# AI4quantum/qiskit-gym

Hardware: AMD Instinct MI355X
Metric: env-steps/sec (whole node), CliffordGym 16q x 65536 envs/GPU; bit-exact vs CPU (higher is better)
Workload: dtype u32

## Files before the change

### qiskit_gym_amd/csrc/kernels_qm.hip

```cpp
#include <cstdlib>

#include "device_common.hpp"
#include "qgym_plan.hpp"
#include "qm_step1.hpp"

namespace qg {


template <int NXP, bool HAS_Z>
struct QmRows {
    static constexpr int R = HAS_Z ? 2 * NXP : NXP;
    static constexpr int G = R / 4;
    static constexpr int xs(int j) { return HAS_Z ? 2 * j : j; }
    static constexpr int zs(int j) { return 2 * j + 1; }
    uint32_t r[R];
};

template <int NXP, bool HAS_Z>
__device__ inline void qm_load(const uint4 *tile, uint32_t lane, QmRows<NXP, HAS_Z> &s) {
#pragma unroll
    for (int g = 0; g < QmRows<NXP, HAS_Z>::G; ++g) {
        const uint4 q = tile[g * 64 + lane];
        s.r[4 * g + 0] = q.x; s.r[4 * g + 1] = q.y; s.r[4 * g + 2] = q.z; s.r[4 * g + 3] = q.w;
    }
// ... 202 lines not shown
        v[i] = i < R ? 1u << i : 0u;
    }
    uint32_t singular = 0;
#pragma unroll 1
    for (int col = 0; col < R; ++col) {
        uint32_t pm = 0, pv = 0;
#pragma unroll
        for (int k = 0; k < 32; ++k) {
            pm = (k == col) ? m[k] : pm;
            pv = (k == col) ? v[k] : pv;
        }
        uint32_t need = ((pm >> col) & 1u) - 1u;
#pragma unroll
        for (int r = 0; r < 32; ++r) {
            const uint32_t t = (r > col && r < R) ? (need & (0u - ((m[r] >> col) & 1u))) : 0u;
            pm ^= m[r] & t;
            pv ^= v[r] & t;
            need &= ~t;
        }
        singular |= need;
#pragma unroll
        for (int r = 0; r < 32; ++r) {
            const uint32_t t = (r != col && r < R) ? (0u - ((m[r] >> col) & 1u)) : 0u;
            m[r] = (r == col) ? pm : (m[r] ^ (pm & t));
            v[r] = (r == col) ? pv : (v[r] ^ (pv & t));
        }
    }
    if (singular) return false;
#pragma unroll
    for (int i = 0; i < 32; ++i) {
        const bool pad = i < R && (uint32_t)(i % NXP) >= N;
        if (pad) v[i] = 0;
    }
    if constexpr (HAS_Z) {
        qm_from_slot_space<NXP>(s, N, v);
    } else {
#pragma unroll
        for (int i = 0; i < R; ++i) s.r[i] = v[i];
    }
    return true;
}

template <int NXP>
__device__ inline void qm_symplectic_inverse(QmRows<NXP, true> &s, uint32_t N) {
    uint32_t m[32], c[32];
    qm_to_slot_space<NXP>(s, N, m);
    qm_symplectic_candidate<NXP>(m, c);
    qm_from_slot_space<NXP>(s, N, c);
}

template <int NXP>
__device__ inline bool qm_check_symplectic(const QmRows<NXP, true> &s, uint32_t N) {
    uint32_t m[32], c[32];
    qm_to_slot_space<NXP>(s, N, m);
    qm_symplectic_candidate<NXP>(m, c);
    return qm_is_inverse<NXP>(m, c, N);
}

template <int NXP, bool HAS_Z, bool FEAT, bool SEQ, bool INV = false, bool GJ = false>
__global__ __launch_bounds__(256) void qm_step_kernel(StepArgs a) {
    using Rows = QmRows<NXP, HAS_Z>;
    const uint64_t env = (uint64_t)blockIdx.x * blockDim.x + threadIdx.x;
    const uint32_t lane = threadIdx.x & (QG_WAVE - 1);
    const bool valid = env < a.B;
    const bool act64 = a.flags & F_ACT64;
    uint4 *tile = reinterpret_cast<uint4 *>(a.state) + (env >> 6) * (uint64_t)(Rows::G * 64);

    if (!valid) return;
    int64_t act = load_action(a.actions, env, act64);
    Rows s;
    qm_load<NXP, HAS_Z>(tile, lane, s);
    int32_t depth = a.depth[env];
    uint32_t iflags = INV ? a.inverted[env] : 0u;

    uint32_t dirty = 0;
    bool solved = false;
    float reward = 0.0f;
    uint32_t fault = 0;
    int32_t sol_n = (FEAT && (a.flags & F_TRACK)) ? a.sol_len[env * 2] : 0;
    int32_t sol_b = (FEAT && INV && (a.flags & F_TRACK)) ? a.sol_len[env * 2 + 1] : 0;

    const uint32_t T = SEQ ? a.T : 1u;
    for (uint32_t t = 0; t < T; ++t) {
        if (SEQ && t) act = load_action(a.actions, (uint64_t)t * a.B + env, act64);
        const bool in_range = act >= 0 && act < (int64_t)a.num_actions;
        GateEntry g = {QM_IDENTITY << 10, 0.0f};
        if (in_range) g = a.gates[act];
        float penalty = g.penalty;
        if (FEAT && (a.flags & F_LAYERS) && in_range)
            penalty = layers_penalty(layer_rec(a.layers, env, 2 * a.N + 2), a.N, a.descs[act], a.w);

        dirty |= qm_apply<NXP, HAS_Z>(s, g.ops);

        if (FEAT && (a.flags & F_TRACK)) {
            if ((uint32_t)(sol_n + sol_b) < a.sol_cap) {
                const bool inv_frame = INV && (iflags & QM_FLAG_INVERTED);
                sol_at(a, env, (uint32_t)(sol_n + sol_b)) = sol_word_framed(act, inv_frame);
                if (inv_frame) ++sol_b;
                else ++sol_n;
            } else {
                fault |= 8u;
            }
        }
        depth = depth > 0 ? depth - 1 : 0;
        if constexpr (INV) {
            const uint32_t coin = a.coins ? a.coins[(uint64_t)t * a.B + env]
                                          : (uint32_t)(rng_draw(a.seed ^ 0x636F696Eull, a.env_base + env, step_clock(a) + t) >> 63);
            if (coin & 1u) {
                bool fast = false;
                if constexpr (HAS_Z) {
                    if (iflags & QM_FLAG_SYMPLECTIC) {
                        qm_symplectic_inverse<NXP>(s, a.N);
                        fast = true;
                    }
                }
                if (fast) {
                    iflags ^= QM_FLAG_INVERTED;
                    dirty = 0xFFFFFFFFu;
                } else if constexpr (GJ) {
                    if (qm_gauss_jordan<NXP, HAS_Z>(s, a.N)) {
                        iflags ^= QM_FLAG_INVERTED;
                        dirty = 0xFFFFFFFFu;
                    } else {
                        fault |= QG_FAULT_SINGULAR;
                    }
                } else {
                    fault |= QG_FAULT_BAD_STATE;
                }
            }
        }
        solved = qm_solved<NXP, HAS_Z>(s, a.N);
        const float achieved = solved ? 1.0f : 0.0f;
        reward = achieved - penalty;
        if (SEQ && a.rewards_seq) a.rewards_seq[(uint64_t)t * a.B + env] = reward;
        if (SEQ && a.dones_seq) a.dones_seq[(uint64_t)t * a.B + env] = (uint8_t)(depth == 0 || solved);
    }

#pragma unroll
    for (int g = 0; g < Rows::G; ++g)
        if ((dirty >> g) & 1u) tile[g * 64 + lane] = make_uint4(s.r[4 * g], s.r[4 * g + 1], s.r[4 * g + 2], s.r[4 * g + 3]);
    a.depth[env] = depth;
    a.reward[env] = reward;
    a.done[env] = (uint8_t)(depth == 0 || solved);
    a.success[env] = (uint8_t)solved;
    if (FEAT && (a.flags & F_TRACK)) {
        a.sol_len[env * 2] = sol_n;
        if (INV) a.sol_len[env * 2 + 1] = sol_b;
    }
    if (INV) a.inverted[env] = (uint8_t)iflags;
    if ((FEAT || INV) && fault) atomicOr(&a.error[env], fault);
    if (a.bad) a.bad[env] = qm_badmask<NXP, HAS_Z>(s, a.N);
}

template <int NXP, bool FEAT, bool LIST = false, bool DENSE = false>
__global__ __launch_bounds__(256) void qm_inv2_kernel(StepArgs a) {
    KernelClock kclk(a.kclk, a.kclk_waves);
    const uint64_t tid = (uint64_t)blockIdx.x * blockDim.x + threadIdx.x;
    __shared__ uint32_t dense_rows[DENSE ? 4 : 1][DENSE ? 32 * 33 : 1];
    uint32_t *dl = DENSE ? dense_rows[threadIdx.x >> 6] : nullptr;
    QG_PREFETCH_STEP_ARGS(a);
    bool whole = false;
    if constexpr (LIST || DENSE) {
        bool fin = false;
        if ((tid >> 1) < a.B) fin = qm_inv2_body<NXP / 2, FEAT, DENSE>(a, NXP / 2, tid >> 1, (uint32_t)tid & 1u, nullptr, dl, &whole);
        if constexpr (DENSE) qm_inv2_dense_flush(a.dense, dl, (tid - (threadIdx.x & 63u)) >> 1, whole);
        if constexpr (LIST) done_mask_store_pairs(a.done_mask, a.B, fin, tid, a.done_epoch);
    } else {
        if ((tid >> 1) >= a.B) return;
        (void)qm_inv2_body<NXP / 2, FEAT, DENSE>(a, NXP / 2, tid >> 1, (uint32_t)tid & 1u, nullptr, dl, &whole);
    }
}


template <int NXP, bool HAS_Z, bool ACT64>
__global__ __launch_bounds__(256) void qm_fused_lds_kernel(StepArgs a) {
    using Rows = QmRows<NXP, HAS_Z>;
    __shared__ uint32_t lds_rows[4][Rows::R][QG_WAVE];
    const uint64_t env = (uint64_t)blockIdx.x * blockDim.x + threadIdx.x;
    const uint32_t lane = threadIdx.x & (QG_WAVE - 1);
    if (env >= a.B) return;
    uint32_t (*rows)[QG_WAVE] = lds_rows[threadIdx.x >> 6];
    uint4 *tile = reinterpret_cast<uint4 *>(a.state) + (env >> 6) * (uint64_t)(Rows::G * 64);
    uint32_t bad;
    {
        Rows s;
        qm_load<NXP, HAS_Z>(tile, lane, s);
        bad = qm_badmask<NXP, HAS_Z>(s, a.N);
#pragma unroll
        for (int k = 0; k < Rows::R; ++k) rows[k][lane] = s.r[k];
    }
    int32_t depth = a.depth[env];
    const uint32_t zb = 1u << a.N;
    float reward = 0.0f;
    bool solved = bad == 0;
    auto load_act = [&](uint32_t t) -> int64_t {
        const uint64_t i = (uint64_t)(t < a.T ? t : a.T - 1u) * a.B + env;
        const int64_t v = ACT64 ? reinterpret_cast<const int64_t *>(a.actions)[i] : (int64_t) reinterpret_cast<const int32_t *>(a.actions)[i];
        return t < a.T ? v : -1;
    };
    auto load_gate = [&](int64_t act, GateEntry &g) {
        const bool ok = act >= 0 && act < (int64_t)a.num_actions;
        const GateEntry e = a.gates[ok ? act : 0];
        g.ops = ok ? e.ops : (QM_IDENTITY << 10);
        g.penalty = ok ? e.penalty : 0.0f;
    };
    auto step = [&](uint32_t t, const GateEntry &g) {
        if (t >= a.T) return;
        const uint32_t q0 = g.ops & 31u, q1 = (g.ops >> 5) & 31u, m = (g.ops >> 10) & 0xFFFFu;
        if (m != QM_IDENTITY) {
            const uint32_t sx0 = HAS_Z ? 2u * q0 : q0, sx1 = HAS_Z ? 2u * q1 : q1;
            const uint32_t x0 = rows[sx0][lane], x1 = rows[sx1][lane];
            const uint32_t z0 = HAS_Z ? rows[sx0 + 1u][lane] : 0u, z1 = HAS_Z ? rows[sx1 + 1u][lane] : 0u;
            auto mix = [&](uint32_t k) -> uint32_t {
                const uint32_t b = m >> (4 * k);
                uint32_t o = ((0u - (b & 1u)) & x0) ^ ((0u - ((b >> 2) & 1u)) & x1);
                if (HAS_Z) o ^= ((0u - ((b >> 1) & 1u)) & z0) ^ ((0u - ((b >> 3) & 1u)) & z1);
                return o;
            };
            const uint32_t nx0 = mix(0), nx1 = mix(2), nz0 = HAS_Z ? mix(1) : 0u, nz1 = HAS_Z ? mix(3) : 0u;
            rows[sx1][lane] = nx1;
            if (HAS_Z) rows[sx1 + 1u][lane] = nz1;
            rows[sx0][lane] = nx0;
            if (HAS_Z) rows[sx0 + 1u][lane] = nz0;
            const uint32_t b1 = (uint32_t)(nx1 != (1u << q1) || (HAS_Z && nz1 != (zb << q1)));
            const uint32_t b0 = (uint32_t)(nx0 != (1u << q0) || (HAS_Z && nz0 != (zb << q0)));
            bad = (bad & ~(1u << q1)) | (b1 << q1);
            bad = (bad & ~(1u << q0)) | (b0 << q0);
        }
        depth = depth > 0 ? depth - 1 : 0;
        solved = bad == 0;
        const float achieved = solved ? 1.0f : 0.0f;
        reward = achieved - g.penalty;
        if (a.rewards_seq) a.rewards_seq[(uint64_t)t * a.B + env] = reward;
        if (a.dones_seq) a.dones_seq[(uint64_t)t * a.B + env] = (uint8_t)(depth == 0 || solved);
    };
    GateEntry cur[4], nxt[4];
    int64_t acts[4];
#pragma unroll
    for (uint32_t k = 0; k < 4; ++k) load_gate(load_act(k), cur[k]);
#pragma unroll
    for (uint32_t k = 0; k < 4; ++k) acts[k] = load_act(4 + k);
    for (uint32_t t = 0; t < a.T; t += 4) {
#pragma unroll
        for (uint32_t k = 0; k < 4; ++k) load_gate(acts[k], nxt[k]);
#pragma unroll
        for (uint32_t k = 0; k < 4; ++k) acts[k] = load_act(t + 8 + k);
#pragma unroll
        for (uint32_t k = 0; k < 4; ++k) step(t + k, cur[k]);
#pragma unroll
        for (uint32_t k = 0; k < 4; ++k) cur[k] = nxt[k];
    }
#pragma unroll
    for (int g = 0; g < Rows::G; ++g)
        tile[g * 64 + lane] = make_uint4(rows[4 * g][lane], rows[4 * g + 1][lane], rows[4 * g + 2][lane], rows[4 * g + 3][lane]);
    a.depth[env] = depth;
    a.reward[env] = reward;
    a.done[env] = (uint8_t)(depth == 0 || solved);
    a.success[env] = (uint8_t)solved;
    if (a.bad) a.bad[env] = bad;
}

__device__ inline uint32_t qm_slot(uint32_t row, uint32_t N, uint32_t nxp, bool has_z) {
    (void)nxp;
    return has_z ? (row < N ? 2 * row : 2 * (row - N) + 1) : row;
}

template <int NXP, bool HAS_Z, bool RESET_ONLY = false>
__device__ inline void qm_init_finish(const InitArgs &a, uint64_t env, const QmRows<NXP, HAS_Z> &s) {
    using Rows = QmRows<NXP, HAS_Z>;
    const uint32_t lane = (uint32_t)(env & (QG_WAVE - 1));
    uint4 *tile = reinterpret_cast<uint4 *>(a.state) + (env >> 6) * (uint64_t)(Rows::G * 64);
    const bool solved = qm_solved<NXP, HAS_Z>(s, a.N);
#pragma unroll
    for (int g = 0; g < Rows::G; ++g) tile[g * 64 + lane] = make_uint4(s.r[4 * g], s.r[4 * g + 1], s.r[4 * g + 2], s.r[4 * g + 3]);
    if (a.bad) a.bad[env] = qm_badmask<NXP, HAS_Z>(s, a.N);
    if constexpr (Rows::R % 16 == 0) {
        if (a.dense) {
#pragma unroll
            for (int k = 0; k < Rows::R; ++k) {
                const uint32_t row = HAS_Z ? ((k & 1) ? a.N + (k >> 1) : (k >> 1)) : (uint32_t)k;
                dense_row_store<Rows::R / 16>(a.dense, env, row, s.r[k]);
            }
        }
    }
    a.depth[env] = a.depth_value;
    a.success[env] = (uint8_t)solved;
    a.reward[env] = solved ? 1.0f : 0.0f;
    a.done[env] = (uint8_t)(a.depth_value == 0 || solved);
    uint32_t symp = 0;
    if constexpr (HAS_Z) {
        if (a.check_symplectic) {
            bool is_symp = true;
            if constexpr (!RESET_ONLY) is_symp = a.mode != 1 || qm_check_symplectic<NXP>(s, a.N);
            symp = is_symp ? QM_FLAG_SYMPLECTIC : 0u;
            if (!symp && a.nonsymp_flag) atomicOr(a.nonsymp_flag, 1u);
        }
    }
    a.inverted[env] = (uint8_t)symp;
    a.error[env] = 0;
    a.sol_len[env * 2] = 0;
    a.sol_len[env * 2 + 1] = 0;
    if (a.layers) {
        const LayerRec lay = layer_rec(a.layers, env, a.layers_len);
        for (uint32_t i = 0; i + 2 < a.layers_len; ++i) lay[i] = -1;
        lay[a.layers_len - 2] = 0;
        lay[a.layers_len - 1] = 0;
    }
}
// ... 451 lines not shown
                const uint32_t slot = 4u * g + c;
                int32_t row;
                if (has_z) row = (slot >> 1) < a.N ? (int32_t)((slot & 1u) ? a.N + (slot >> 1) : (slot >> 1)) : -1;
                else row = slot < a.N ? (int32_t)slot : -1;
                if (row >= 0) my[lane * pitch + (uint32_t)row] = w[c];
            }
        }
    }
    __syncthreads();
    if (tile_idx >= n_tiles) return;
    const uint64_t env0 = tile_idx * 64u;
    const uint32_t envs = a.B - env0 < 64u ? (uint32_t)(a.B - env0) : 64u;
    uint32_t *out = reinterpret_cast<uint32_t *>(a.out) + env0 * D;
    if ((D & 3u) == 0 && (reinterpret_cast<uintptr_t>(out) & 15u) == 0) {
        const uint32_t n4 = envs * D / 4u;
        for (uint32_t i = lane; i < n4; i += 64u) {
            const uint32_t e = (4u * i) / D, r = (4u * i) % D;
            const uint32_t *p = my + e * pitch + r;
            reinterpret_cast<uint4 *>(out)[i] = make_uint4(p[0], p[1], p[2], p[3]);
        }
    } else {
        const uint32_t n = envs * D;
        for (uint32_t i = lane; i < n; i += 64u) out[i] = my[(i / D) * pitch + (i % D)];
    }
}

template <int D16>
__global__ __launch_bounds__(256) void qm_dense_stream_kernel(ObsArgs a, uint32_t has_z) {
    KernelClock kclk(a.kclk, a.kclk_waves);
    constexpr uint32_t D = 16u * D16, G = D / 4u, PITCH = D + 1u, CPE = D * D16;
    __shared__ uint32_t lds[4][64 * PITCH];
    const uint32_t lane = threadIdx.x & 63u, wave = threadIdx.x >> 6;
    const uint64_t n_tiles = (a.B + 63u) / 64u;
    const uint64_t tile_idx = (uint64_t)blockIdx.x * 4u + wave;
    if (tile_idx >= n_tiles) return;
    uint32_t *my = lds[wave];
    const uint4 *tile = reinterpret_cast<const uint4 *>(a.state) + tile_idx * (uint64_t)(G * 64u);
    uint4 vs[G];
#pragma unroll
    for (uint32_t g = 0; g < G; ++g) vs[g] = tile[g * 64u + lane];
#pragma unroll
    for (uint32_t g = 0; g < G; ++g) {
        const uint32_t w[4] = {vs[g].x, vs[g].y, vs[g].z, vs[g].w};
#pragma unroll
        for (uint32_t c = 0; c < 4; ++c) {
            const uint32_t slot = 4u * g + c;
            const uint32_t row = has_z ? ((slot & 1u) ? D / 2u + (slot >> 1) : (slot >> 1)) : slot;
            my[lane * PITCH + row] = w[c];
        }
    }
    __builtin_amdgcn_wave_barrier();
    const uint64_t env0 = tile_idx * 64u;
    const uint32_t envs = a.B - env0 < 64u ? (uint32_t)(a.B - env0) : 64u;
    uint4 *out = reinterpret_cast<uint4 *>(reinterpret_cast<int8_t *>(a.out) + env0 * (uint64_t)(D * D));
    const uint32_t n_chunks = envs * CPE;
#pragma unroll 8
    for (uint32_t i = lane; i < n_chunks; i += 64u) {
        const uint32_t e = i / CPE, r = (i % CPE) / D16, part = i % D16;
        out[i] = expand16_i8(my[e * PITCH + r] >> (16u * part));
    }
}

__global__ __launch_bounds__(256) void qm_dense_stream_any_kernel(ObsArgs a, uint32_t nxp, uint32_t has_z) {
    constexpr uint32_t PITCH = 33u;
    __shared__ uint32_t lds[4][64 * PITCH];
    const uint32_t lane = threadIdx.x & 63u, wave = threadIdx.x >> 6;
    const uint64_t n_tiles = (a.B + 63u) / 64u;
    const uint64_t tile_idx = (uint64_t)blockIdx.x * 4u + wave;
    if (tile_idx >= n_tiles) return;
    uint32_t *my = lds[wave];
    const uint32_t N = a.N, D = a.D, DD = D * D, R = has_z ? 2u * nxp : nxp, G = R / 4u;
    const uint4 *tile = reinterpret_cast<const uint4 *>(a.state) + tile_idx * (uint64_t)(G * 64u);
    uint4 vs[8];
#pragma unroll
    for (uint32_t g = 0; g < 8; ++g) vs[g] = g < G ? tile[g * 64u + lane] : make_uint4(0u, 0u, 0u, 0u);
#pragma unroll
    for (uint32_t g = 0; g < 8; ++g) {
        if (g >= G) break;
        const uint32_t w[4] = {vs[g].x, vs[g].y, vs[g].z, vs[g].w};
#pragma unroll
        for (uint32_t c = 0; c < 4; ++c) {
            const uint32_t slot = 4u * g + c, j = has_z ? slot >> 1 : slot;
            if (j < N) my[lane * PITCH + ((has_z && (slot & 1u)) ? N + j : j)] = w[c];
        }
    }
    __builtin_amdgcn_wave_barrier();
    const uint64_t env0 = tile_idx * 64u;
    const uint32_t envs = a.B - env0 < 64u ? (uint32_t)(a.B - env0) : 64u;
    uint8_t *out = reinterpret_cast<uint8_t *>(a.out) + env0 * (uint64_t)DD;
    const uint32_t n_bytes = envs * DD;
    uint32_t f = 16u * lane;
    uint32_t e = f / DD, rem = f - e * DD, r = rem / D, c = rem - r * D;
    const uint32_t adv_e = 1024u / DD, adv_rem = 1024u - adv_e * DD, adv_r = adv_rem / D, adv_c = adv_rem - adv_r * D;
    for (; f < n_bytes; f += 1024u) {
        uint32_t bits = 0, filled = 0, pe = e, pr = r, pc = c;
        while (filled < 16u && pe < envs) {
            const uint32_t take = (16u - filled) < (D - pc) ? (16u - filled) : (D - pc);
            bits |= ((my[pe * PITCH + pr] >> pc) & ((1u << take) - 1u)) << filled;
            filled += take;
            pc = 0;
            if (++pr == D) {
                pr = 0;
                ++pe;
            }
        }
        const uint4 v = expand16_i8(bits);
        if (n_bytes - f >= 16u) {
            *reinterpret_cast<uint4 *>(out + f) = v;
        } else {
            const uint32_t o[4] = {v.x, v.y, v.z, v.w};
            for (uint32_t b = 0; b < n_bytes - f; ++b) out[f + b] = (uint8_t)(o[b >> 2] >> (8u * (b & 3u)));
        }
        c += adv_c;
        if (c >= D) {
            c -= D;
            ++r;
        }
        r += adv_r;
        if (r >= D) {
            r -= D;
            ++e;
        }
        e += adv_e;
    }
}

template <int ES>
__global__ __launch_bounds__(256) void qm_dense_typed_kernel(const uint32_t *state, uint64_t B, uint32_t N, uint32_t D, uint32_t nxp,
                                                             uint32_t has_z, uint32_t chunks_per_row, uint4 *out, uint32_t one) {
    constexpr uint32_t EPC = 16 / ES;
    const uint64_t gid = (uint64_t)blockIdx.x * blockDim.x + threadIdx.x;
    const uint64_t grow = gid / chunks_per_row;
    const uint64_t env = grow / D;
    if (env >= B) return;
    const uint32_t row = (uint32_t)(grow - env * D), c0 = (uint32_t)(gid - grow * chunks_per_row) * EPC;
    const uint32_t R = has_z ? 2 * nxp : nxp, slot = qm_slot(row, N, nxp, has_z);
    const uint32_t *tile = state + (env >> 6) * (uint64_t)(R * 64);
    const uint32_t w = tile[((slot >> 2) * 64 + (uint32_t)(env & 63)) * 4 + (slot & 3)];
    out[gid] = expand_chunk<ES>((w >> c0) & ((1u << EPC) - 1u), one);
}

static inline unsigned grid_for(uint64_t threads, unsigned block) { return (unsigned)((threads + block - 1) / block); }

template <int NXP, bool HAS_Z>
static hipError_t launch_step(const StepArgs &a, hipStream_t s) {
    const dim3 grid(grid_for(a.B, 256)), block(256);
    const bool feat = a.flags & (F_TRACK | F_LAYERS);
    const bool seq = a.T != 1 || a.rewards_seq || a.dones_seq;
    const bool list = a.flags & F_DONE_LIST;
    switch (plan::tile_step(false, plan::tile_inv_kernels(false, HAS_Z, NXP), a.flags, a.T, a.bad != nullptr, a.rewards_seq || a.dones_seq, a.num_actions)) {
    case plan::SK_QM_STEP1: return qm_step1(a, NXP, HAS_Z, s);
    case plan::SK_QM_INV2:
        if constexpr (HAS_Z && NXP <= 16) {
            const dim3 grid2(grid_for(2 * a.B, 256)), lgrid2 = grid2, lblock = block;
            if constexpr (NXP == 16) {
                if (a.dense) {
                    if (feat && list) hipLaunchKernelGGL((qm_inv2_kernel<NXP, true, true, true>), lgrid2, lblock, 0, s, a);
                    else if (feat) hipLaunchKernelGGL((qm_inv2_kernel<NXP, true, false, true>), grid2, block, 0, s, a);
                    else if (list) hipLaunchKernelGGL((qm_inv2_kernel<NXP, false, true, true>), lgrid2, lblock, 0, s, a);
                    else hipLaunchKernelGGL((qm_inv2_kernel<NXP, false, false, true>), grid2, block, 0, s, a);
                    return hipGetLastError();
                }
            }
            if (feat && list) hipLaunchKernelGGL((qm_inv2_kernel<NXP, true, true>), lgrid2, lblock, 0, s, a);
            else if (feat) hipLaunchKernelGGL((qm_inv2_kernel<NXP, true>), grid2, block, 0, s, a);
            else if (list) hipLaunchKernelGGL((qm_inv2_kernel<NXP, false, true>), lgrid2, lblock, 0, s, a);
            else hipLaunchKernelGGL((qm_inv2_kernel<NXP, false>), grid2, block, 0, s, a);
            return hipGetLastError();
        }
        return hipErrorInvalidValue;
    case plan::SK_QM_STEP_GJ:
        if constexpr (HAS_Z && NXP <= 16) {
            hipLaunchKernelGGL((qm_step_kernel<NXP, HAS_Z, true, true, true, true>), grid, block, 0, s, a);
            return hipGetLastError();
        }
        return hipErrorInvalidValue;
    case plan::SK_QM_STEP_INV:
        if constexpr (HAS_Z && NXP <= 16) {
            hipLaunchKernelGGL((qm_step_kernel<NXP, HAS_Z, true, true, true, false>), grid, block, 0, s, a);
            return hipGetLastError();
        }
        return hipErrorInvalidValue;
    case plan::SK_QM_FUSED_LDS:
        if (a.flags & F_ACT64) hipLaunchKernelGGL((qm_fused_lds_kernel<NXP, HAS_Z, true>), grid, block, 0, s, a);
        else hipLaunchKernelGGL((qm_fused_lds_kernel<NXP, HAS_Z, false>), grid, block, 0, s, a);
        return hipGetLastError();
    case plan::SK_QM_STEP:
        if (feat && seq) hipLaunchKernelGGL((qm_step_kernel<NXP, HAS_Z, true, true>), grid, block, 0, s, a);
        else if (feat) hipLaunchKernelGGL((qm_step_kernel<NXP, HAS_Z, true, false>), grid, block, 0, s, a);
        else if (seq) hipLaunchKernelGGL((qm_step_kernel<NXP, HAS_Z, false, true>), grid, block, 0, s, a);
        else hipLaunchKernelGGL((qm_step_kernel<NXP, HAS_Z, false, false>), grid, block, 0, s, a);
        return hipGetLastError();
    default: return hipErrorInvalidValue;
    }
}
template <int NXP, bool HAS_Z>
static hipError_t launch_init(const InitArgs &a, hipStream_t s) {
    const bool lean = a.mode == 2 && a.list;
    uint64_t threads = lean ? 4 * a.B : a.B;
    if (a.list && a.coop && a.n_draws >= 64u) {
        const uint64_t tree_blocks = a.tree_grid;
        if (tree_blocks * QG_TREE_THREADS > threads) threads = tree_blocks * QG_TREE_THREADS;
    }
    if (lean) hipLaunchKernelGGL((qm_init_kernel<NXP, HAS_Z, 1>), dim3(grid_for(threads, 256)), dim3(256), 0, s, a);
    else if (a.mode == 2) hipLaunchKernelGGL((qm_init_kernel<NXP, HAS_Z, 2>), dim3(grid_for(threads, 256)), dim3(256), 0, s, a);
    else hipLaunchKernelGGL((qm_init_kernel<NXP, HAS_Z>), dim3(grid_for(threads, 256)), dim3(256), 0, s, a);
    return hipGetLastError();
}

#define QM_DISPATCH(FN, ARGS)                                         \
    if (has_z) {                                                      \
        switch (nxp) {                                                \
        case 4: return FN<4, true>(ARGS, s);                          \
        case 8: return FN<8, true>(ARGS, s);                          \
        case 12: return FN<12, true>(ARGS, s);                        \
        case 16: return FN<16, true>(ARGS, s);                        \
        }                                                             \
    } else {                                                          \
        switch (nxp) {                                                \
        case 4: return FN<4, false>(ARGS, s);                         \
        case 8: return FN<8, false>(ARGS, s);                         \
        case 12: return FN<12, false>(ARGS, s);                       \
        case 16: return FN<16, false>(ARGS, s);                       \
        case 20: return FN<20, false>(ARGS, s);                       \
        case 24: return FN<24, false>(ARGS, s);                       \
        case 28: return FN<28, false>(ARGS, s);                       \
        case 32: return FN<32, false>(ARGS, s);                       \
        }                                                             \
    }                                                                 \
    return hipErrorInvalidValue;

hipError_t qm_step(const StepArgs &a, uint32_t nxp, bool has_z, hipStream_t s) {
    if (!a.B) return hipSuccess;
    QM_DISPATCH(launch_step, a)
}
hipError_t qm_init(const InitArgs &a, uint32_t nxp, bool has_z, hipStream_t s) {
    if (!a.B) return hipSuccess;
    QM_DISPATCH(launch_init, a)
}
template <int NXP, bool HAS_Z>
static hipError_t launch_reset_step(const ResetStepArgs &ra, hipStream_t s) {
    const InitArgs &ia = ra.reset;
    uint64_t threads = 4 * ia.B;
    uint64_t tree_blocks = 0;
    if (ia.list && ia.coop && ia.n_draws >= plan::TREE_MIN_DRAWS) {
        tree_blocks = ia.tree_grid;
        if (tree_blocks * QG_TREE_THREADS > threads) threads = tree_blocks * QG_TREE_THREADS;
    }
    ResetStepArgs rb = ra;
    rb.reset_blocks = grid_for(threads, 256);
    rb.first_reset = tree_blocks ? (uint32_t)std::min<uint64_t>(tree_blocks, rb.reset_blocks) : rb.reset_blocks / 2;
    const bool feat = ra.step.flags & (F_TRACK | F_LAYERS), layers = ra.step.flags & F_LAYERS;
    if (ra.step.flags & F_INVERTS) {
        if constexpr (HAS_Z && NXP <= 16) {
            rb.step_blocks = grid_for(2 * ra.step.B, 256);
            const dim3 grid2(rb.reset_blocks + rb.step_blocks);
            if (ra.step.flags & F_LAYERS) hipLaunchKernelGGL((qm_reset_inv2_step_kernel<NXP, true, false>), grid2, dim3(256), 0, s, rb);
            else if (feat) hipLaunchKernelGGL((qm_reset_inv2_step_kernel<NXP, true, true>), grid2, dim3(256), 0, s, rb);
            else hipLaunchKernelGGL((qm_reset_inv2_step_kernel<NXP, false, true>), grid2, dim3(256), 0, s, rb);
            return hipGetLastError();
        }
        return hipErrorInvalidValue;
    }
    rb.step_blocks = grid_for(ra.step.B, 256);
    const dim3 grid(rb.reset_blocks + rb.step_blocks), block(256);
    if constexpr (QmRows<NXP, HAS_Z>::R % 16 == 0) {
        if (ra.step.dense) {
            if (layers) hipLaunchKernelGGL((qm_reset_step_kernel<NXP, HAS_Z, true, true, false>), grid, block, 0, s, rb);
            else if (feat) hipLaunchKernelGGL((qm_reset_step_kernel<NXP, HAS_Z, true, true, true>), grid, block, 0, s, rb);
            else hipLaunchKernelGGL((qm_reset_step_kernel<NXP, HAS_Z, false, true>), grid, block, 0, s, rb);
            return hipGetLastError();
        }
    }
    if (layers) hipLaunchKernelGGL((qm_reset_step_kernel<NXP, HAS_Z, true, false, false>), grid, block, 0, s, rb);
    else if (feat) hipLaunchKernelGGL((qm_reset_step_kernel<NXP, HAS_Z, true, false, true>), grid, block, 0, s, rb);
    else hipLaunchKernelGGL((qm_reset_step_kernel<NXP, HAS_Z, false, false>), grid, block, 0, s, rb);
    return hipGetLastError();
}
hipError_t qm_reset_step(const InitArgs &reset, const StepArgs &step, uint32_t nxp, bool has_z, hipStream_t s) {
    if (!step.B) return hipSuccess;
    ResetStepArgs ra;
    ra.reset = reset;
    ra.step = step;
    ra.reset_blocks = ra.step_blocks = ra.first_reset = 0;
    QM_DISPATCH(launch_reset_step, ra)
}

hipError_t qm_export(const ObsArgs &a, uint32_t nxp, bool has_z, hipStream_t s) {
    if (!a.B) return hipSuccess;
    const uint32_t R = has_z ? 2 * nxp : nxp;
    const uintptr_t addr = reinterpret_cast<uintptr_t>(a.out);
    switch (plan::tile_export(a.format, a.D, R, a.out_stride, (addr & 15) == 0, (addr & 3) == 0)) {
    case plan::EK_DENSE_STREAM: {
        const dim3 grid((unsigned)((a.B + 255) / 256)), block(256);
        if (a.D == 32) hipLaunchKernelGGL(qm_dense_stream_kernel<2>, grid, block, 0, s, a, has_z ? 1u : 0u);
        else hipLaunchKernelGGL(qm_dense_stream_kernel<1>, grid, block, 0, s, a, has_z ? 1u : 0u);
        return hipGetLastError();
    }
    case plan::EK_DENSE_STREAM_ANY:
        hipLaunchKernelGGL(qm_dense_stream_any_kernel, dim3((unsigned)((a.B + 255) / 256)), dim3(256), 0, s, a, nxp, has_z ? 1u : 0u);
        return hipGetLastError();
    case plan::EK_PACK:
        hipLaunchKernelGGL(qm_pack_kernel, dim3((unsigned)((a.B + 255) / 256)), dim3(256), 0, s, a, nxp, has_z ? 1u : 0u);
        return hipGetLastError();
    default: break;
    }
    hipLaunchKernelGGL(qm_export_kernel, dim3(grid_for(a.B * a.D, 256)), dim3(256), 0, s, a, nxp, has_z ? 1u : 0u);
    return hipGetLastError();
}

hipError_t qm_export_typed(const void *state, uint64_t B, uint32_t N, uint32_t D, uint32_t nxp, bool has_z, void *out, uint32_t es,
                           uint32_t one, hipStream_t s) {
    if (!B) return hipSuccess;
    const uint32_t cpr = D / (16 / es);
    if (cpr == 0 || D % (16 / es) != 0) return hipErrorInvalidValue;
    const dim3 grid(grid_for(B * D * cpr, 256)), block(256);
    const uint32_t *st = reinterpret_cast<const uint32_t *>(state);
    uint4 *o = reinterpret_cast<uint4 *>(out);
    if (es == 1) hipLaunchKernelGGL(qm_dense_typed_kernel<1>, grid, block, 0, s, st, B, N, D, nxp, has_z ? 1u : 0u, cpr, o, one);
    else if (es == 2) hipLaunchKernelGGL(qm_dense_typed_kernel<2>, grid, block, 0, s, st, B, N, D, nxp, has_z ? 1u : 0u, cpr, o, one);
// ... 6 lines not shown
```

### qiskit_gym_amd/csrc/qgym_internal.hpp

```cpp
#pragma once

#include <hip/hip_runtime.h>
#include <stdint.h>

#include "../../include/qgym.h"

namespace qg {

struct GateEntry {
    uint32_t ops;
    float penalty;
};
static_assert(sizeof(GateEntry) == 8, "GateEntry must be 8 bytes");

enum : uint32_t { OP_NONE = 0, OP_XOR = 1, OP_SWAP = 2 };
__host__ __device__ inline uint32_t make_op(uint32_t type, uint32_t dst, uint32_t src) {
    return (dst & 63u) | ((src & 63u) << 6) | ((type & 3u) << 12);
}

__host__ __device__ inline uint32_t make_desc(uint32_t kind, uint32_t q0, uint32_t q1) {
    return (kind & 0xFFu) | ((q0 & 0xFFu) << 8) | ((q1 & 0xFFu) << 16);
}

enum : uint32_t {
// ... 7 lines not shown

__host__ __device__ inline uint64_t done_mask_words(uint64_t B) { return 4ull * ((B + 255ull) / 256ull); }
__host__ __device__ inline uint64_t done_mask_bytes(uint64_t B) { return done_mask_words(B) * 10ull + 8ull; }

__host__ __device__ inline uint64_t splitmix64(uint64_t x) {
    x += 0x9E3779B97F4A7C15ull;
    x = (x ^ (x >> 30)) * 0xBF58476D1CE4E5B9ull;
    x = (x ^ (x >> 27)) * 0x94D049BB133111EBull;
    return x ^ (x >> 31);
}
__host__ __device__ inline uint64_t rng_draw(uint64_t seed, uint64_t env, uint64_t t) {
    return splitmix64(seed ^ splitmix64(env * 0x9E3779B97F4A7C15ull + t));
}
__host__ __device__ inline uint32_t rng_action(uint64_t seed, uint64_t env, uint64_t t, uint32_t num_actions) {
#if defined(__HIP_DEVICE_COMPILE__)
    return (uint32_t)__umul64hi(rng_draw(seed, env, t), (uint64_t)num_actions);
#else
    return (uint32_t)(((unsigned __int128)rng_draw(seed, env, t) * (unsigned __int128)num_actions) >> 64);
#endif
}

struct StepArgs {
    void *state;
    const void *actions;
    const uint8_t *coins;
    const GateEntry *gates;
    const uint32_t *descs;
    int32_t *depth;
    float *reward;
    uint8_t *done;
    uint8_t *success;
    uint8_t *inverted;
    uint32_t *error;
    uint32_t *sol;
    int32_t *sol_len;
    int32_t *layers;
    float *rewards_seq;
    uint8_t *dones_seq;
    uint64_t B;
    uint64_t seed;
    uint64_t step_index;
    uint32_t D;
    uint32_t N;
    uint32_t log2L;
    uint32_t num_actions;
    uint32_t T;
    uint32_t flags;
    uint32_t sol_cap;
    float w[4];
    float pauli_layer_reward;
    uint32_t max_rotations;
    uint32_t kclk_waves;
    const uint64_t *clock;
    uint64_t env_base;
    uint32_t *bad;
    unsigned long long *kclk;
    uint32_t *done_list;
    uint32_t *done_count;
    int8_t *dense;
    uint64_t *done_mask;
    uint32_t done_epoch;
};

#if defined(__HIP_DEVICE_COMPILE__) && !defined(QG_NO_ARG_PREFETCH)
#define QG_PREFETCH_STEP_ARGS(a)                                                                                                          \
    asm volatile("" ::"s"((a).state), "s"((a).actions), "s"((a).gates), "s"((a).depth), "s"((a).bad), "s"((a).B), "s"((a).flags),        \
                 "s"((a).num_actions), "s"((a).N), "s"((a).rewards_seq), "s"((a).dones_seq), "s"((a).reward), "s"((a).done), "s"((a).success), \
                 "s"((a).kclk))
#else
#define QG_PREFETCH_STEP_ARGS(a) ((void)0)
#endif

constexpr uint64_t QG_COMPACT_MIN_ENVS = 4096;
constexpr uint64_t QG_STREAM_MIN_ENVS = 64;

struct InitArgs {
    void *state;
    int32_t *depth;
    float *reward;
    uint8_t *done;
    uint8_t *success;
    uint8_t *inverted;
    uint32_t *error;
    int32_t *sol_len;
    int32_t *layers;
    const GateEntry *gates;
    const int32_t *actions;
    const void *src;
    uint64_t src_stride;
    uint64_t B;
    uint64_t seed;
    uint32_t D, N, log2L, num_actions;
    uint32_t n_draws;
    int32_t depth_value;
    uint32_t format;
    uint32_t mode;
    uint32_t layers_len;
    uint32_t check_symplectic;
    uint32_t only_done;
    uint32_t flags_current;
    uint32_t *nonsymp_flag;
    const uint64_t *clock;
    uint32_t *bad;
    const uint64_t *mask;
    uint32_t mask_words;
    uint32_t mask_epoch;
    uint32_t *count_pub;
    const uint32_t *list;
    uint32_t *list_count;
    uint32_t tree_grid;
    uint32_t *zero_count;
    uint32_t coop;
    const uint32_t *rowops;
    uint64_t env_base;
    uint32_t inverts;
    int8_t *dense;
    unsigned long long *kclk;
    uint32_t kclk_waves;
    uint32_t *count_out;
};

#define QG_CLOCK_SEED_STRIDE 0x9E3779B9ull
__device__ inline uint64_t clock_of(const uint64_t *c) { return c ? *c : 0ull; }
__device__ inline uint64_t step_clock(const StepArgs &a) { return a.step_index + clock_of(a.clock); }
__device__ inline uint64_t init_seed(const InitArgs &a) { return a.seed + QG_CLOCK_SEED_STRIDE * clock_of(a.clock); }

struct ObsArgs {
    const void *state;
    void *out;
    uint64_t B;
    uint64_t out_stride;
    uint32_t D, N, log2L;
    uint32_t format;
    uint32_t obs_rows, obs_cols;
    unsigned long long *kclk;
    uint32_t kclk_waves;
};

#define QG_FMT_BITS 3u
__device__ inline uint64_t bits_window(const uint64_t *bs, uint64_t pos, uint32_t D) {
    const uint32_t sh = (uint32_t)pos & 63u;
    const uint64_t lo = bs[pos >> 6], hi = bs[(pos >> 6) + 1];
    const uint64_t w = sh ? (lo >> sh) | (hi << (64u - sh)) : lo;
    return D >= 64u ? w : w & ((1ull << D) - 1ull);
}

hipError_t lfd_step(const StepArgs &a, bool w64, uint32_t rg, hipStream_t s);
hipError_t lfd_init(const InitArgs &a, bool w64, uint32_t rg, const uint32_t *descs, hipStream_t s);
hipError_t lfd_export(const ObsArgs &a, bool w64, uint32_t rg, const uint8_t *inverted, hipStream_t s);

hipError_t qm_step(const StepArgs &a, uint32_t nxp, bool has_z, hipStream_t s);
hipError_t qm_init(const InitArgs &a, uint32_t nxp, bool has_z, hipStream_t s);
hipError_t qm_step1(const StepArgs &a, uint32_t nxp, bool has_z, hipStream_t s);
hipError_t qm_reset_step(const InitArgs &reset, const StepArgs &step, uint32_t nxp, bool has_z, hipStream_t s);
hipError_t q64_reset_step(const InitArgs &reset, const StepArgs &step, uint32_t ns, bool has_z, hipStream_t s);
hipError_t qm_export(const ObsArgs &a, uint32_t nxp, bool has_z, hipStream_t s);
hipError_t qm_export_typed(const void *state, uint64_t B, uint32_t N, uint32_t D, uint32_t nxp, bool has_z, void *out, uint32_t elem_size,
                           uint32_t one, hipStream_t s);

hipError_t q64_step(const StepArgs &a, uint32_t ns, bool has_z, hipStream_t s);
hipError_t q64_init(const InitArgs &a, uint32_t ns, bool has_z, hipStream_t s);
hipError_t q64_export(const ObsArgs &a, uint32_t ns, bool has_z, hipStream_t s);

hipError_t lf8_step(const StepArgs &a, bool fused, hipStream_t s);
hipError_t lf8_init(const InitArgs &a, hipStream_t s);
hipError_t lf8_export(const ObsArgs &a, hipStream_t s);

hipError_t word_reset_step(const InitArgs &reset, const StepArgs &step, bool perm, hipStream_t s);
hipError_t perm_step(const StepArgs &a, bool fused, hipStream_t s);
hipError_t perm_init(const InitArgs &a, hipStream_t s);
hipError_t perm_export(const ObsArgs &a, hipStream_t s);
hipError_t permb_step(const StepArgs &a, uint32_t ng, hipStream_t s);
hipError_t permb_init(const InitArgs &a, uint32_t ng, const uint32_t *descs, hipStream_t s);
hipError_t permb_export(const ObsArgs &a, uint32_t ng, hipStream_t s);

hipError_t expand_rows(const void *words_dev, int word_bytes, uint64_t n_rows, uint32_t cols, void *out_dev, int out_dtype, hipStream_t s);
hipError_t expand_rows_i64(const void *words_dev, int word_bytes, uint64_t n_rows, uint32_t cols, int64_t *out_dev, hipStream_t s);
hipError_t pack_bitstream(const void *src, int elem_bytes, uint64_t n_entries, uint64_t *out_words, hipStream_t s);
hipError_t compact_done(const uint8_t *done, uint64_t B, uint32_t *list, uint32_t *count, hipStream_t s);

constexpr uint32_t COPY_MAX_REGIONS = 16;
struct CopyRegionArgs {
    char *dst;
    const char *src;
    uint64_t tile_bytes;
    uint64_t pitch_dst, pitch_src;
    uint32_t rows, w;
};
struct CopyArgs {
    CopyRegionArgs r[COPY_MAX_REGIONS];
    uint32_t n_regions;
    const uint32_t *src_idx;
    const uint32_t *dst_idx;
    uint64_t n, B_src, B_dst;
    int8_t *dense;
    uint32_t D, N, has_z;
};
hipError_t copy_envs(const CopyArgs &a, hipStream_t s);
hipError_t masks_fill(const uint8_t *success, uint8_t *out, uint64_t B, uint32_t num_actions, hipStream_t s);
hipError_t fault_any(const uint32_t *error, uint64_t B, uint32_t *scratch, uint32_t *out_host, hipStream_t s);
hipError_t step_outputs(const float *reward, const uint8_t *done, const uint8_t *success, float *rewards_out, uint8_t *dones_out, uint8_t *success_out,
                        uint64_t B, hipStream_t s);

}
```

Measured before the change: 24.44 billion.

## Split plain inv2 kernel into dedicated file with branchless gate masks

Moves the non-list, non-dense inv2 step into its own translation unit, with a new body. The body passes hot pointers as scalar kernel arguments, issues the action, gate and sol_len loads early behind scheduling barriers, and replaces per-qubit selects with branchless bit-mask selection, dirtying per row pair. The symplectic inversion butterfly is rewritten with a scalar mask. The aim is to cut front-end load latency and VALU/branch cost, at the price of a second code path with ablation macros to maintain.

```diff
diff --git a/qiskit_gym_amd/csrc/kernels_qm.hip b/qiskit_gym_amd/csrc/kernels_qm.hip
--- a/qiskit_gym_amd/csrc/kernels_qm.hip
+++ b/qiskit_gym_amd/csrc/kernels_qm.hip
@@ -378,8 +378,9 @@
     if (a.bad) a.bad[env] = qm_badmask<NXP, HAS_Z>(s, a.N);
 }
 
-template <int NXP, bool FEAT, bool LIST = false, bool DENSE = false>
+template <int NXP, bool FEAT, bool LIST, bool DENSE>
 __global__ __launch_bounds__(256) void qm_inv2_kernel(StepArgs a) {
+    static_assert(LIST || DENSE, "the plain instantiations: kernels_qm_inv2.hip");
     KernelClock kclk(a.kclk, a.kclk_waves);
     const uint64_t tid = (uint64_t)blockIdx.x * blockDim.x + threadIdx.x;
     __shared__ uint32_t dense_rows[DENSE ? 4 : 1][DENSE ? 32 * 33 : 1];
@@ -1137,20 +1138,19 @@
     case plan::SK_QM_STEP1: return qm_step1(a, NXP, HAS_Z, s);
     case plan::SK_QM_INV2:
         if constexpr (HAS_Z && NXP <= 16) {
-            const dim3 grid2(grid_for(2 * a.B, 256)), lgrid2 = grid2, lblock = block;
+            const dim3 grid2(grid_for(2 * a.B, 256));
             if constexpr (NXP == 16) {
                 if (a.dense) {
-                    if (feat && list) hipLaunchKernelGGL((qm_inv2_kernel<NXP, true, true, true>), lgrid2, lblock, 0, s, a);
+                    if (feat && list) hipLaunchKernelGGL((qm_inv2_kernel<NXP, true, true, true>), grid2, block, 0, s, a);
                     else if (feat) hipLaunchKernelGGL((qm_inv2_kernel<NXP, true, false, true>), grid2, block, 0, s, a);
-                    else if (list) hipLaunchKernelGGL((qm_inv2_kernel<NXP, false, true, true>), lgrid2, lblock, 0, s, a);
+                    else if (list) hipLaunchKernelGGL((qm_inv2_kernel<NXP, false, true, true>), grid2, block, 0, s, a);
                     else hipLaunchKernelGGL((qm_inv2_kernel<NXP, false, false, true>), grid2, block, 0, s, a);
                     return hipGetLastError();
                 }
             }
-            if (feat && list) hipLaunchKernelGGL((qm_inv2_kernel<NXP, true, true>), lgrid2, lblock, 0, s, a);
-            else if (feat) hipLaunchKernelGGL((qm_inv2_kernel<NXP, true>), grid2, block, 0, s, a);
-            else if (list) hipLaunchKernelGGL((qm_inv2_kernel<NXP, false, true>), lgrid2, lblock, 0, s, a);
-            else hipLaunchKernelGGL((qm_inv2_kernel<NXP, false>), grid2, block, 0, s, a);
+            if (!list) return qm_inv2(a, NXP, s);
+            if (feat) hipLaunchKernelGGL((qm_inv2_kernel<NXP, true, true, false>), grid2, block, 0, s, a);
+            else hipLaunchKernelGGL((qm_inv2_kernel<NXP, false, true, false>), grid2, block, 0, s, a);
             return hipGetLastError();
         }
         return hipErrorInvalidValue;
diff --git a/qiskit_gym_amd/csrc/kernels_qm_inv2.hip b/qiskit_gym_amd/csrc/kernels_qm_inv2.hip
--- /dev/null
+++ b/qiskit_gym_amd/csrc/kernels_qm_inv2.hip
@@ -0,0 +1,48 @@
+#include "device_common.hpp"
+#include "qgym_plan.hpp"
+#include "qm_inv2.hpp"
+
+namespace qg {
+
+constexpr uint32_t QM_INV2_BLOCK = 256;
+
+template <int NXP, bool FEAT, bool LIST = false, bool DENSE = false>
+__global__ __launch_bounds__(QM_INV2_BLOCK) void qm_inv2_kernel(const void *actions, void *state, int32_t *depth, uint8_t *inverted, const uint8_t *coins,
+                                                                 uint64_t B, uint32_t flags, uint32_t num_actions, StepArgs a) {
+    static_assert(!LIST && !DENSE, "the LIST and DENSE instantiations: kernels_qm.hip");
+#if QG_INV2_ABLATE & 1
+    const uint32_t block = blockDim.x;
+    KernelClock kclk(a.kclk, a.kclk_waves);
+    QG_PREFETCH_STEP_ARGS(a);
+    const Inv2Front f = inv2_front(a);
+#else
+    constexpr uint32_t block = QM_INV2_BLOCK;
+    KernelClock kclk(a.kclk, a.kclk_waves, QM_INV2_BLOCK);
+    const Inv2Front f{actions, state, depth, inverted, coins, B, flags, num_actions};
+#endif
+    const uint64_t tid = (uint64_t)blockIdx.x * block + threadIdx.x;
+    if ((tid >> 1) >= f.B) return;
+    (void)qm_inv2_masks_body<NXP / 2, FEAT>(f, a, tid >> 1, (uint32_t)tid & 1u);
+}
+
+template <int NXP>
+static hipError_t launch_inv2(const StepArgs &a, hipStream_t s) {
+    const dim3 grid((unsigned)((2 * a.B + QM_INV2_BLOCK - 1) / QM_INV2_BLOCK)), block(QM_INV2_BLOCK);
+    const bool feat = a.flags & (F_TRACK | F_LAYERS);
+    if (feat) hipLaunchKernelGGL((qm_inv2_kernel<NXP, true>), grid, block, 0, s, a.actions, a.state, a.depth, a.inverted, a.coins, a.B, a.flags, a.num_actions, a);
+    else hipLaunchKernelGGL((qm_inv2_kernel<NXP, false>), grid, block, 0, s, a.actions, a.state, a.depth, a.inverted, a.coins, a.B, a.flags, a.num_actions, a);
+    return hipGetLastError();
+}
+
+hipError_t qm_inv2(const StepArgs &a, uint32_t nxp, hipStream_t s) {
+    if (!a.B) return hipSuccess;
+    switch (nxp) {
+    case 4: return launch_inv2<4>(a, s);
+    case 8: return launch_inv2<8>(a, s);
+    case 12: return launch_inv2<12>(a, s);
+    case 16: return launch_inv2<16>(a, s);
+    }
+    return hipErrorInvalidValue;
+}
+
+}
diff --git a/qiskit_gym_amd/csrc/qgym_internal.hpp b/qiskit_gym_amd/csrc/qgym_internal.hpp
--- a/qiskit_gym_amd/csrc/qgym_internal.hpp
+++ b/qiskit_gym_amd/csrc/qgym_internal.hpp
@@ -183,6 +183,7 @@
 hipError_t qm_step(const StepArgs &a, uint32_t nxp, bool has_z, hipStream_t s);
 hipError_t qm_init(const InitArgs &a, uint32_t nxp, bool has_z, hipStream_t s);
 hipError_t qm_step1(const StepArgs &a, uint32_t nxp, bool has_z, hipStream_t s);
+hipError_t qm_inv2(const StepArgs &a, uint32_t nxp, hipStream_t s);
 hipError_t qm_reset_step(const InitArgs &reset, const StepArgs &step, uint32_t nxp, bool has_z, hipStream_t s);
 hipError_t q64_reset_step(const InitArgs &reset, const StepArgs &step, uint32_t ns, bool has_z, hipStream_t s);
 hipError_t qm_export(const ObsArgs &a, uint32_t nxp, bool has_z, hipStream_t s);
diff --git a/qiskit_gym_amd/csrc/qm_inv2.hpp b/qiskit_gym_amd/csrc/qm_inv2.hpp
--- /dev/null
+++ b/qiskit_gym_amd/csrc/qm_inv2.hpp
@@ -0,0 +1,262 @@
+#pragma once
+
+#include "qm_step1.hpp"
+
+namespace qg {
+
+#ifndef QG_INV2_ABLATE
+#define QG_INV2_ABLATE 0
+#endif
+
+struct Inv2Front {
+    const void *actions;
+    void *state;
+    int32_t *depth;
+    uint8_t *inverted;
+    const uint8_t *coins;
+    uint64_t B;
+    uint32_t flags, num_actions;
+};
+__device__ inline Inv2Front inv2_front(const StepArgs &a) { return Inv2Front{a.actions, a.state, a.depth, a.inverted, a.coins, a.B, a.flags, a.num_actions}; }
+
+__device__ inline void inv2_butterfly(uint32_t &lo, uint32_t &hi, uint32_t d, uint32_t m) {
+    const uint32_t l = lo, u = hi;
+    lo = bit_select(m, l, u << d);
+    hi = bit_select(m, l >> d, u);
+}
+
+template <int GS, bool FEAT>
+__device__ inline bool qm_inv2_masks_body(const Inv2Front &f, const StepArgs &a, uint64_t env, uint32_t h) {
+    constexpr int G = GS;
+    constexpr bool NEW_FRONT = !(QG_INV2_ABLATE & 1), NEW_ALU = !(QG_INV2_ABLATE & 2), NEW_INV = !(QG_INV2_ABLATE & 4);
+    uint4 *tile = reinterpret_cast<uint4 *>(f.state) + (env >> 6) * (uint64_t)(G * 64) + (env & 63u);
+    int32_t act_lo = 0, act_hi = 0;
+    if constexpr (NEW_FRONT) action_issue(f.actions, env, f.flags & F_ACT64, act_lo, act_hi);
+    uint4 grp[4];
+#pragma unroll
+    for (int k = 0; k < 4; ++k) {
+        grp[k] = make_uint4(0u, 0u, 0u, 0u);
+        if (k < G && (h == 0 || k + 4 < G)) grp[k] = tile[(uint32_t)(4 * h + k) * 64u];
+    }
+    int32_t depth = f.depth[env];
+    uint32_t iflags = f.inverted[env];
+    uint32_t coin;
+    int32_t sol_n = 0, sol_b = 0;
+    int64_t act;
+    bool in_range;
+    GateEntry g;
+    uintptr_t out_reward = 0, out_done = 0, out_success = 0;
+    if constexpr (NEW_FRONT) {
+        coin = (f.coins ? f.coins : f.inverted)[env];
+        __builtin_amdgcn_sched_barrier(0);
+        asm volatile("" : : "s"(a.gates), "s"(a.N), "s"(a.rewards_seq), "s"(a.dones_seq), "s"(a.reward), "s"(a.done), "s"(a.success), "s"(a.kclk_waves));
+        if constexpr (FEAT) asm volatile("" : : "s"(a.sol), "s"(a.sol_cap), "s"(a.sol_len));
+        __builtin_amdgcn_sched_barrier(0);
+        act = action_value(act_lo, act_hi, f.flags & F_ACT64);
+        in_range = (uint64_t)act < (uint64_t)f.num_actions;
+        uint32_t gi = in_range ? (uint32_t)act : 0u;
+        asm volatile("" : "+v"(gi));
+        const GateEntry entry = a.gates[gi];
+        __builtin_amdgcn_sched_barrier(0);
+        if constexpr (FEAT) {
+            const int2 sl = *reinterpret_cast<const int2 *>(a.sol_len + env * 2);
+            sol_n = sl.x; sol_b = sl.y;
+        }
+        out_reward = reinterpret_cast<uintptr_t>(a.reward + env); out_done = reinterpret_cast<uintptr_t>(a.done + env);
+        out_success = reinterpret_cast<uintptr_t>(a.success + env);
+        asm volatile("" : "+v"(out_reward), "+v"(out_done), "+v"(out_success));
+        if (!f.coins) coin = (uint32_t)(rng_draw(a.seed ^ 0x636F696Eull, a.env_base + env, step_clock(a)) >> 63);
+        g = entry;
+        if (!in_range) g = GateEntry{QM_IDENTITY << 10, 0.0f};
+    } else {
+        coin = f.coins ? f.coins[env] : 0u;
+        sol_n = (FEAT && (f.flags & F_TRACK)) ? a.sol_len[env * 2] : 0;
+        sol_b = (FEAT && (f.flags & F_TRACK)) ? a.sol_len[env * 2 + 1] : 0;
+        act = load_action(f.actions, env, f.flags & F_ACT64);
+        in_range = act >= 0 && act < (int64_t)f.num_actions;
+        g = a.gates[in_range ? act : 0];
+        if (!in_range) g = GateEntry{QM_IDENTITY << 10, 0.0f};
+        if (!f.coins) coin = (uint32_t)(rng_draw(a.seed ^ 0x636F696Eull, a.env_base + env, step_clock(a)) >> 63);
+    }
+    const uint32_t N = a.N;
+    uint32_t xs[8], zs[8];
+#pragma unroll
+    for (int k = 0; k < 4; ++k) {
+        xs[2 * k] = grp[k].x; zs[2 * k] = grp[k].y; xs[2 * k + 1] = grp[k].z; zs[2 * k + 1] = grp[k].w;
+    }
+    uint32_t fault = 0;
+    float penalty = g.penalty;
+    if (FEAT && (f.flags & F_LAYERS) && in_range && h == 0) penalty = layers_penalty(layer_rec(a.layers, env, 2 * N + 2), N, a.descs[act], a.w);
+
+    uint32_t dirty = 0;
+    constexpr uint32_t ALL_DIRTY = NEW_ALU ? 0xFFu : 0xFu;
+    auto group_dirty = [&](int k) -> bool { return NEW_ALU ? (dirty & (3u << (2 * k))) != 0u : ((dirty >> k) & 1u) != 0u; };
+    const uint32_t q0 = g.ops & 31u, q1 = (g.ops >> 5) & 31u, m = (g.ops >> 10) & 0xFFFFu;
+    const bool live = m != QM_IDENTITY;
+    uint32_t nx0, nz0, nx1, nz1;
+    if constexpr (NEW_ALU) {
+        const uint32_t ops = g.ops, hm = 0u - h;
+        uint32_t mm[16];
+#pragma unroll
+        for (uint32_t i = 0; i < 16; ++i) mm[i] = gate_bit_mask(ops, 10u + i);
+        const uint32_t w0 = ~(gate_bit_mask(ops, 3u) ^ hm), w1 = ~(gate_bit_mask(ops, 8u) ^ hm);
+        auto pick = [&](uint32_t b0, uint32_t b1, uint32_t b2, uint32_t own, uint32_t &x, uint32_t &z) {
+            const uint32_t ux = bit_select(b2, bit_select(b1, grp[3].x, grp[2].x), bit_select(b1, grp[1].x, grp[0].x));
+            const uint32_t uy = bit_select(b2, bit_select(b1, grp[3].y, grp[2].y), bit_select(b1, grp[1].y, grp[0].y));
+            const uint32_t uz = bit_select(b2, bit_select(b1, grp[3].z, grp[2].z), bit_select(b1, grp[1].z, grp[0].z));
+            const uint32_t uw = bit_select(b2, bit_select(b1, grp[3].w, grp[2].w), bit_select(b1, grp[1].w, grp[0].w));
+            x = own & bit_select(b0, uz, ux);
+            z = own & bit_select(b0, uw, uy);
+            x |= qm_pair_swap(x); z |= qm_pair_swap(z);
+        };
+        uint32_t x0, z0, x1, z1;
+        pick(gate_bit_mask(ops, 0u), gate_bit_mask(ops, 1u), gate_bit_mask(ops, 2u), w0, x0, z0);
+        pick(gate_bit_mask(ops, 5u), gate_bit_mask(ops, 6u), gate_bit_mask(ops, 7u), w1, x1, z1);
+        auto mix = [&](uint32_t k) -> uint32_t {
+            return xor_and(xor_and(xor_and(mm[4 * k] & x0, mm[4 * k + 1], z0), mm[4 * k + 2], x1), mm[4 * k + 3], z1);
+        };
+        nx0 = mix(0); nz0 = mix(1); nx1 = mix(2); nz1 = mix(3);
+        const uint32_t lv = (uint32_t)live;
+        const uint32_t hot0 = (w0 & lv) << (q0 & 7u), hot1 = (w1 & lv) << (q1 & 7u);
+#pragma unroll
+        for (uint32_t j = 0; j < 8; ++j) {
+            const uint32_t e0 = gate_bit_mask(hot0, j), e1 = gate_bit_mask(hot1, j);
+            xs[j] = bit_select(e0, nx0, bit_select(e1, nx1, xs[j]));
+            zs[j] = bit_select(e0, nz0, bit_select(e1, nz1, zs[j]));
+        }
+        dirty = hot0 | hot1;
+    } else {
+        const bool own0 = (q0 >> 3) == h, own1 = (q1 >> 3) == h;
+        uint32_t x0 = own0 ? tree_select<8>(xs, q0 & 7u) : 0u, z0 = own0 ? tree_select<8>(zs, q0 & 7u) : 0u;
+        uint32_t x1 = own1 ? tree_select<8>(xs, q1 & 7u) : 0u, z1 = own1 ? tree_select<8>(zs, q1 & 7u) : 0u;
+        x0 |= qm_pair_swap(x0); z0 |= qm_pair_swap(z0);
+        x1 |= qm_pair_swap(x1); z1 |= qm_pair_swap(z1);
+        auto mix = [&](uint32_t k) -> uint32_t {
+            const uint32_t b = m >> (4 * k);
+            return ((0u - (b & 1u)) & x0) ^ ((0u - ((b >> 1) & 1u)) & z0) ^ ((0u - ((b >> 2) & 1u)) & x1) ^ ((0u - ((b >> 3) & 1u)) & z1);
+        };
+        nx0 = mix(0); nz0 = mix(1); nx1 = mix(2); nz1 = mix(3);
+        if (live) {
+#pragma unroll
+            for (int j = 0; j < 8; ++j) {
+                const bool h1 = own1 && (q1 & 7u) == (uint32_t)j, h0 = own0 && (q0 & 7u) == (uint32_t)j;
+                uint32_t vx = xs[j], vz = zs[j];
+                vx = h1 ? nx1 : vx; vz = h1 ? nz1 : vz;
+                vx = h0 ? nx0 : vx; vz = h0 ? nz0 : vz;
+                xs[j] = vx; zs[j] = vz;
+            }
+            if (own0) dirty |= 1u << ((q0 & 7u) >> 1);
+            if (own1) dirty |= 1u << ((q1 & 7u) >> 1);
+        }
+    }
+
+    if (FEAT && (f.flags & F_TRACK) && h == 0) {
+        if ((uint32_t)(sol_n + sol_b) < a.sol_cap) {
+            const bool inv_frame = iflags & QM_FLAG_INVERTED;
+            sol_at(a, env, (uint32_t)(sol_n + sol_b)) = sol_word_framed(act, inv_frame);
+            if (inv_frame) ++sol_b;
+            else ++sol_n;
+        } else {
+            fault |= 8u;
+        }
+    }
+    depth = depth > 0 ? depth - 1 : 0;
+
+    if (coin & 1u) {
+        if (iflags & QM_FLAG_SYMPLECTIC) {
+            uint32_t w[16];
+            const uint32_t xm = N >= 16 ? 0xFFFFu : ((1u << N) - 1u);
+#pragma unroll
+            for (int j = 0; j < 8; ++j) {
+                w[j] = xs[j];
+                w[8 + j] = zs[j];
+            }
+            if (N < 16) {
+#pragma unroll
+                for (int i = 0; i < 16; ++i) w[i] = (w[i] & xm) | (((w[i] >> N) & xm) << 16);
+            }
+#pragma unroll
+            for (int st = 0; st < 3; ++st) {
+                const int d = 4 >> st;
+                uint32_t mlo = st == 0 ? 0x0F0F0F0Fu : st == 1 ? 0x33333333u : 0x55555555u;
+                if constexpr (NEW_INV) asm volatile("" : "+s"(mlo));
+#pragma unroll
+                for (int i = 0; i < 16; ++i) {
+                    if ((i & d) == 0) {
+                        if constexpr (NEW_INV) {
+                            inv2_butterfly(w[i], w[i + d], (uint32_t)d, mlo);
+                        } else {
+                            const uint32_t lo = w[i], hi = w[i + d];
+                            w[i] = (lo & mlo) | ((hi & mlo) << d);
+                            w[i + d] = ((lo >> d) & mlo) | (hi & ~mlo);
+                        }
+                    }
+                }
+            }
+            const uint32_t sel8 = h ? 0x03070105u : 0x06020400u;
+#pragma unroll
+            for (int i = 0; i < 16; ++i) w[i] = __builtin_amdgcn_perm(qm_pair_swap(w[i]), w[i], sel8);
+#pragma unroll
+            for (int j = 0; j < 8; ++j) {
+                const uint32_t lo = w[j], hi = w[8 + j];
+                w[j] = __builtin_amdgcn_perm(hi, lo, 0x03020706u);
+                w[8 + j] = __builtin_amdgcn_perm(hi, lo, 0x01000504u);
+            }
+            if (N < 16) {
+#pragma unroll
+                for (int i = 0; i < 16; ++i) w[i] = (w[i] & xm) | (((w[i] >> 16) & xm) << N);
+            }
+#pragma unroll
+            for (int j = 0; j < 8; ++j) {
+                xs[j] = w[j];
+                zs[j] = w[8 + j];
+            }
+            iflags ^= QM_FLAG_INVERTED;
+            dirty = ALL_DIRTY;
+        } else {
+            fault |= QG_FAULT_BAD_STATE;
+        }
+    }
+
+    uint32_t diff = 0;
+#pragma unroll
+    for (int j = 0; j < 8; ++j) {
+        const uint32_t q = 8u * h + (uint32_t)j;
+        const bool real = q < N;
+        diff |= xs[j] ^ (real ? 1u << q : 0u);
+        diff |= zs[j] ^ (real ? (1u << N) << q : 0u);
+    }
+    diff |= qm_pair_swap(diff);
+    const bool solved = diff == 0;
+    const float achieved = solved ? 1.0f : 0.0f;
+    const float reward = achieved - penalty;
+
+#pragma unroll
+    for (int k = 0; k < 4; ++k)
+        if (group_dirty(k) && k < G && (h == 0 || k + 4 < G))
+            tile[(uint32_t)(4 * h + k) * 64u] = make_uint4(xs[2 * k], zs[2 * k], xs[2 * k + 1], zs[2 * k + 1]);
+    const bool fin = depth == 0 || solved;
+    if (h == 0) {
+        if (a.rewards_seq) a.rewards_seq[env] = reward;
+        if (a.dones_seq) a.dones_seq[env] = (uint8_t)fin;
+        f.depth[env] = depth;
+        if constexpr (NEW_FRONT) {
+            global_store(out_reward, reward);
+            global_store(out_done, (uint8_t)fin);
+            global_store(out_success, (uint8_t)solved);
+        } else {
+            a.reward[env] = reward;
+            a.done[env] = (uint8_t)fin;
+            a.success[env] = (uint8_t)solved;
+        }
+        if (FEAT && (f.flags & F_TRACK)) {
+            a.sol_len[env * 2] = sol_n;
+            a.sol_len[env * 2 + 1] = sol_b;
+        }
+        f.inverted[env] = (uint8_t)iflags;
+        if (fault) atomicOr(&a.error[env], fault);
+    }
+    return fin;
+}
+
+}
```

New measurement: 24.50 billion (median of 2 runs). About the same (+0.2%).
